# renjie-liang/HUAL

Measured on AMD Instinct MI355X. Metric: train clips/sec, higher is better.
Workload: dtype f32 (fp16x3 / bf16x3 split-operand MFMA, fp32 accumulate); 1 GPU; Charades-STA SeqPAN train step (fwd+bwd+clip+AdamWD, dropout 0.2), batch 64/GPU, T=128, vdim=1024, L=20, C=8, dim=128, 8 heads, 2 attention layers, random init; ONE batch resident in HBM, batch assembly (hual_assemble_batch) outside the timed region; global_batch=64, T=128, vdim=1024, L=20, parallelism=dp1, launch=hipGraph, video_dtype=f32

## Files before the change

hual_amd/csrc/heads.h:

```cpp
#pragma once
#include "common.h"
#include "rowops.h"

namespace hual {

enum { LA_MATCH_SUM = 0, LA_MASK_SUM = 1, LA_ORTHO = 2, LA_LOC = 3, LA_ALIGN = 4, LA_DENOM = 5 };

struct PoolArgs {
  const float* F2;
  const float* wp;
  const float* Wbot;
  float* alpha;
  float* pooled;
  float* PW;
};
struct AlignPool;
struct AlignPoolBwd;
int launch_pool_align_fwd(const PoolArgs& a, const AlignPool* ap, const RowSpace& rs, hipStream_t s);
struct PoolBwd {
  const float* dFuse;
  float* dPW;
  float* dF2;
  float* dwp;
};
int launch_pool_align_bwd(const PoolArgs& a, const PoolBwd& g, const AlignPool& ap, const AlignPoolBwd& ab, const RowSpace& rs, hipStream_t s);

struct MatchArgs {
  const float* fuse;
  const float* Wm;
  const float* bm;
  const float* E;
  const int32_t* labels;
  float* probs;
  float* probs2;
  float* outputs;
  float* loss_acc;
  float* part;
  const uint32_t* rng;
  float inv_tau;
};
int match_fwd_blocks(int Nv);
struct AlignSim;
int launch_match_fwd(const MatchArgs& a, const RowSpace& rs, const AlignSim* as, hipStream_t s);
struct LossTailArgs {
  float* loss_acc; const float* match_part; int match_nblk; const float* loc_part; int loc_nblk;
  float lambda, override_denom; const float* denom_dev; float* loss_out;
  const uint32_t* ovf; int novf;
  const float* align_rows; int nalign;
};
struct MatchBwd {
  const float* dOut;
  const float* dOut2;
  float* dFuse;
  float* dWm; float* dbm; float* dE;
  const float* dE_ortho;
  float* part;
  float lambda;
  int do_tail; LossTailArgs tail;
};
int match_bwd_blocks(int Nv);
int launch_match_bwd(const MatchArgs& a, const MatchBwd& g, const RowSpace& rs, hipStream_t s);
struct HeadsArgs {
  const float* h[2]; const float* w[2]; const float* b[2];
  float* logit[2];
  const float* vmask;
  const float* y1; const float* y2;
  int64_t* start_index; int64_t* end_index;
  float* ds; float* de;
  int grad_only;
  float* dZ[2];
  float* part[2];
  float* loc_part;
  float inv_batch;
  const uint32_t* ovf; int novf;
};
int launch_heads(const HeadsArgs& a, int B, int T, hipStream_t s);
int launch_loss_tail(const LossTailArgs& a, hipStream_t s);

struct AlignPool {
  const float* F2;
  const float* F1;
  const float* inner;
  float* tpre; float* vpre;
  float* that; float* vhat;
  int ld;
};
struct AlignSim {
  const float* that; const float* vhat; int Bg;
  float* dq; float* da;
  float* row_loss;
  float* dthat; float* dvhat;
  float* loss_acc;
  float scale;
  int ld;
  int row0, nrows;
};
int launch_align_sim(const AlignSim& a, hipStream_t s);
struct AlignPoolBwd {
  const float* dthat; const float* dvhat;
  float* dF2;
  float* dF1;
  const float* col_dq; const float* col_da; int col_Bg;
};

}
```

hual_amd/csrc/heads.hip:

```cpp
#include "heads.h"
#include "philox.h"
#include "prof.h"

using namespace hual;

#if defined(HUAL_STAMPS) && HUAL_STAMPS == 8
static __device__ unsigned long long g_heads_stamps[512 * 64];
extern "C" int hual_debug_stamps(unsigned long long* out, int n) {
  return (int)hipMemcpyFromSymbol(out, HIP_SYMBOL(g_heads_stamps), sizeof(unsigned long long) * (size_t)n);
}
#define HEADS_STAMP(i) do { if (threadIdx.x == 0 && blockIdx.x < 512) g_heads_stamps[blockIdx.x * 64 + (i)] = __builtin_readcyclecounter(); } while (0)
#else
#define HEADS_STAMP(i) do { } while (0)
#endif

__device__ __forceinline__ void pool_fwd_body(const PoolArgs& a, const RowSpace& rs, int b) {
  __shared__ float al[256];
  __shared__ float pooled[HUAL_D];
  __shared__ float part[HUAL_D];
  const int tid = threadIdx.x;
  const bool on = tid < 256;
  const int l32 = tid & 31, grp = tid >> 5;
  const int L = rs.L;
  const float* F = a.F2 + (size_t)(rs.Nv + b * L) * HUAL_D;
  const float* m = rs.rowmask + rs.Nv + b * L;
  if (on) {
    const float4 w4 = ld4(a.wp + 4 * l32);
    for (int l = grp; l < L; l += 8) {
      const float4 f = ld4(F + (size_t)l * HUAL_D + 4 * l32);
      const float d = fast_sum32(f.x * w4.x + f.y * w4.y + f.z * w4.z + f.w * w4.w);
      if (l32 == 0) al[l] = d * m[l] + HUAL_MASK_VALUE * (1.0f - m[l]);
    }
  }
  __syncthreads();
  float mx = -INFINITY;
  for (int l = 0; l < L; ++l) mx = fmaxf(mx, al[l]);
  float sum = 0.f;
  for (int l = 0; l < L; ++l) sum += __expf(al[l] - mx);
  const float inv = 1.0f / sum;
  const int c = tid & 127, half = (tid >> 7) & 1;
  if (on && half == 0) {
    float p = 0.f;
    for (int l = 0; l < L; ++l) {
      const float alpha = __expf(al[l] - mx) * inv;
      if (c == 0) a.alpha[b * L + l] = alpha;
      p = fmaf(alpha, F[(size_t)l * HUAL_D + c], p);
    }
    pooled[c] = p;
    a.pooled[b * HUAL_D + c] = p;
  }
  __syncthreads();
  float o = 0.f;
  if (on) {
#pragma unroll 8
// ... 15 lines not shown
  float ce_sum = 0.f, m_sum = 0.f;
  float4 w0 = ld4(a.Wm + (col + 0) * 4), w1 = ld4(a.Wm + (col + 1) * 4), w2 = ld4(a.Wm + (col + 2) * 4), w3 = ld4(a.Wm + (col + 3) * 4);
  const float4 bm = ld4(a.bm);
  float4 e0 = ld4(a.E + col), e1 = ld4(a.E + HUAL_D + col), e2 = ld4(a.E + 2 * HUAL_D + col), e3 = ld4(a.E + 3 * HUAL_D + col);
  uint3 gk = make_uint3(0u, 0u, 0u);
  if (a.rng) gk = make_uint3(a.rng[0], a.rng[1], a.rng[2]);
  for (int row = bid * 8 + grp; row < rs.Nv; row += nblk * 8) {
    const size_t off = (size_t)row * HUAL_D + col;
    const float4 f = ld4(a.fuse + off);
    float l0 = f.x * w0.x + f.y * w1.x + f.z * w2.x + f.w * w3.x;
    float l1 = f.x * w0.y + f.y * w1.y + f.z * w2.y + f.w * w3.y;
    float l2 = f.x * w0.z + f.y * w1.z + f.z * w2.z + f.w * w3.z;
    float l3 = f.x * w0.w + f.y * w1.w + f.z * w2.w + f.w * w3.w;
    l0 = fast_sum32(l0) + bm.x; l1 = fast_sum32(l1) + bm.y; l2 = fast_sum32(l2) + bm.z; l3 = fast_sum32(l3) + bm.w;
    if (a.rng) {
      const uint4_ r = philox4x32(0u, (uint32_t)row, (uint32_t)HUAL_SITE_GUMBEL, gk.z, gk.x, gk.y);
      l0 = (l0 + gumbel_noise(r.x)) * a.inv_tau; l1 = (l1 + gumbel_noise(r.y)) * a.inv_tau;
      l2 = (l2 + gumbel_noise(r.z)) * a.inv_tau; l3 = (l3 + gumbel_noise(r.w)) * a.inv_tau;
    }
    const float mx = fmaxf(fmaxf(l0, l1), fmaxf(l2, l3));
    const float x0 = expf(l0 - mx), x1 = expf(l1 - mx), x2 = expf(l2 - mx), x3 = expf(l3 - mx);
    const float sum = x0 + x1 + x2 + x3;
    const float inv = 1.0f / sum;
    const float p0 = x0 * inv, p1 = x1 * inv, p2 = x2 * inv, p3 = x3 * inv;
    const float mk = rs.rowmask[row];
    if (l32 == 0) {
      *reinterpret_cast<float4*>(a.probs + (size_t)row * 4) = make_float4(p0, p1, p2, p3);
      if (a.probs2) *reinterpret_cast<float4*>(a.probs2 + (size_t)row * 4) = make_float4(p0, p1, p2, p3);
      if (a.labels) {
        const int lab = a.labels[row];
        const float ll = lab == 0 ? l0 : (lab == 1 ? l1 : (lab == 2 ? l2 : l3));
        ce_sum += (mx + logf(sum) - ll) * mk;
        m_sum += mk;
      }
    }
    float4 o = make_float4((f.x + p0 * e0.x + p1 * e1.x + p2 * e2.x + p3 * e3.x) * mk,
                           (f.y + p0 * e0.y + p1 * e1.y + p2 * e2.y + p3 * e3.y) * mk,
                           (f.z + p0 * e0.z + p1 * e1.z + p2 * e2.z + p3 * e3.z) * mk,
                           (f.w + p0 * e0.w + p1 * e1.w + p2 * e2.w + p3 * e3.w) * mk);
    st4(a.outputs + off, o);
  }
  if (a.labels && a.loss_acc) {
    if (l32 == 0) { red[0][grp] = ce_sum; red[1][grp] = m_sum; }
    __syncthreads();
    if (threadIdx.x == 0) {
      float c = 0.f, m = 0.f;
      for (int i = 0; i < 8; ++i) { c += red[0][i]; m += red[1][i]; }
      if (a.part) { a.part[2 * bid] = c; a.part[2 * bid + 1] = m; }
      else { atomicAdd(a.loss_acc + LA_MATCH_SUM, c); atomicAdd(a.loss_acc + LA_MASK_SUM, m); }
    }
  }
}

__device__ __forceinline__ float loss_tail_body(const LossTailArgs& a, float* sm, bool write);
__global__ __launch_bounds__(256) void match_bwd_kernel(MatchArgs a, MatchBwd g, RowSpace rs) {
  __shared__ float4 red[8][8][32];
  __shared__ float redb[8][4];
  const int l32 = threadIdx.x & 31, grp = threadIdx.x >> 5;
  const int col = 4 * l32;
  float4 w0 = ld4(a.Wm + (col + 0) * 4), w1 = ld4(a.Wm + (col + 1) * 4), w2 = ld4(a.Wm + (col + 2) * 4), w3 = ld4(a.Wm + (col + 3) * 4);
  float4 e0 = ld4(a.E + col), e1 = ld4(a.E + HUAL_D + col), e2 = ld4(a.E + 2 * HUAL_D + col), e3 = ld4(a.E + 3 * HUAL_D + col);
  const int row0 = min((int)blockIdx.x * 8 + grp, rs.Nv - 1);
  const size_t off0 = (size_t)row0 * HUAL_D + col;
  float pmk = rs.rowmask[row0];
  float4 pd = ld4(g.dOut + off0), pd2 = g.dOut2 ? ld4(g.dOut2 + off0) : f4zero();
  float4 pf = ld4(a.fuse + off0), pp = *reinterpret_cast<const float4*>(a.probs + (size_t)row0 * 4);
  float denom = 1.0f;
  if (g.do_tail) {
    __shared__ float smt[12];
    denom = loss_tail_body(g.tail, smt, blockIdx.x == 0);
  } else if (a.labels) {
    denom = a.loss_acc[LA_DENOM];
  }
  const float ce_scale = a.labels ? g.lambda / denom : 0.f;
  float4 dE0 = f4zero(), dE1 = f4zero(), dE2 = f4zero(), dE3 = f4zero();
  float4 dW0 = f4zero(), dW1 = f4zero(), dW2 = f4zero(), dW3 = f4zero();
  float db0 = 0.f, db1 = 0.f, db2 = 0.f, db3 = 0.f;
  for (int row = blockIdx.x * 8 + grp; row < rs.Nv; row += gridDim.x * 8) {
    const size_t off = (size_t)row * HUAL_D + col;
    const float mk = pmk;
    float4 d = pd;
    if (g.dOut2) d = make_float4(d.x + pd2.x, d.y + pd2.y, d.z + pd2.z, d.w + pd2.w);
    const float4 f = pf, p = pp;
    {
      const int rn = min(row + (int)gridDim.x * 8, rs.Nv - 1);
      const size_t offn = (size_t)rn * HUAL_D + col;
      pmk = rs.rowmask[rn];
      pd = ld4(g.dOut + offn);
      if (g.dOut2) pd2 = ld4(g.dOut2 + offn);
      pf = ld4(a.fuse + offn);
      pp = *reinterpret_cast<const float4*>(a.probs + (size_t)rn * 4);
    }
    d = make_float4(d.x * mk, d.y * mk, d.z * mk, d.w * mk);
    float q0 = fast_sum32(d.x * e0.x + d.y * e0.y + d.z * e0.z + d.w * e0.w);
    float q1 = fast_sum32(d.x * e1.x + d.y * e1.y + d.z * e1.z + d.w * e1.w);
    float q2 = fast_sum32(d.x * e2.x + d.y * e2.y + d.z * e2.z + d.w * e2.w);
    float q3 = fast_sum32(d.x * e3.x + d.y * e3.y + d.z * e3.z + d.w * e3.w);
    const float dot = p.x * q0 + p.y * q1 + p.z * q2 + p.w * q3;
    float dl0 = p.x * (q0 - dot), dl1 = p.y * (q1 - dot), dl2 = p.z * (q2 - dot), dl3 = p.w * (q3 - dot);
    if (a.labels) {
      const int lab = a.labels[row];
      const float cs = ce_scale * mk;
      dl0 += cs * (p.x - (lab == 0 ? 1.f : 0.f));
      dl1 += cs * (p.y - (lab == 1 ? 1.f : 0.f));
      dl2 += cs * (p.z - (lab == 2 ? 1.f : 0.f));
      dl3 += cs * (p.w - (lab == 3 ? 1.f : 0.f));
    }
    if (a.rng) { dl0 *= a.inv_tau; dl1 *= a.inv_tau; dl2 *= a.inv_tau; dl3 *= a.inv_tau; }
    st4(g.dFuse + off, make_float4(d.x + dl0 * w0.x + dl1 * w0.y + dl2 * w0.z + dl3 * w0.w,
                                   d.y + dl0 * w1.x + dl1 * w1.y + dl2 * w1.z + dl3 * w1.w,
                                   d.z + dl0 * w2.x + dl1 * w2.y + dl2 * w2.z + dl3 * w2.w,
                                   d.w + dl0 * w3.x + dl1 * w3.y + dl2 * w3.z + dl3 * w3.w));
    dE0 = make_float4(dE0.x + p.x * d.x, dE0.y + p.x * d.y, dE0.z + p.x * d.z, dE0.w + p.x * d.w);
    dE1 = make_float4(dE1.x + p.y * d.x, dE1.y + p.y * d.y, dE1.z + p.y * d.z, dE1.w + p.y * d.w);
    dE2 = make_float4(dE2.x + p.z * d.x, dE2.y + p.z * d.y, dE2.z + p.z * d.z, dE2.w + p.z * d.w);
    dE3 = make_float4(dE3.x + p.w * d.x, dE3.y + p.w * d.y, dE3.z + p.w * d.z, dE3.w + p.w * d.w);
    dW0 = make_float4(dW0.x + f.x * dl0, dW0.y + f.y * dl0, dW0.z + f.z * dl0, dW0.w + f.w * dl0);
    dW1 = make_float4(dW1.x + f.x * dl1, dW1.y + f.y * dl1, dW1.z + f.z * dl1, dW1.w + f.w * dl1);
    dW2 = make_float4(dW2.x + f.x * dl2, dW2.y + f.y * dl2, dW2.z + f.z * dl2, dW2.w + f.w * dl2);
    dW3 = make_float4(dW3.x + f.x * dl3, dW3.y + f.y * dl3, dW3.z + f.z * dl3, dW3.w + f.w * dl3);
    if (l32 == 0) { db0 += dl0; db1 += dl1; db2 += dl2; db3 += dl3; }
  }
  red[0][grp][l32] = dE0; red[1][grp][l32] = dE1; red[2][grp][l32] = dE2; red[3][grp][l32] = dE3;
  red[4][grp][l32] = dW0; red[5][grp][l32] = dW1; red[6][grp][l32] = dW2; red[7][grp][l32] = dW3;
  if (l32 == 0) { redb[grp][0] = db0; redb[grp][1] = db1; redb[grp][2] = db2; redb[grp][3] = db3; }
  __syncthreads();
  float* part = g.part + (size_t)blockIdx.x * 9 * HUAL_D;
  for (int idx = threadIdx.x; idx < 8 * 128; idx += 256) {
    const int vec = idx >> 7, c = idx & 127;
    float s = 0.f;
#pragma unroll
    for (int k = 0; k < 8; ++k) s += reinterpret_cast<const float*>(&red[vec][k][c >> 2])[c & 3];
    if (vec < 4) {
      if (g.dE_ortho && blockIdx.x == 0) s += g.dE_ortho[vec * HUAL_D + c];
      part[vec * HUAL_D + c] = s;
    } else {
      part[4 * HUAL_D + c * 4 + (vec - 4)] = s;
    }
  }
  if (threadIdx.x < HUAL_D) {
    float s = 0.f;
    if (threadIdx.x < 4)
      for (int k = 0; k < 8; ++k) s += redb[k][threadIdx.x];
    part[8 * HUAL_D + threadIdx.x] = s;
  }
}

template <int NR>
__global__ __launch_bounds__(512) void heads_kernel(HeadsArgs a, int T, int B) {
  __shared__ float zs_[256], ze_[256], ps[256], pe[256], dls[256], dle[256];
  __shared__ float sm[24];
  __shared__ double smd[16];
  __shared__ float wtot[2][4];
  __shared__ float bestv[2][4];
  __shared__ int besti[2][4];
  __shared__ float4 red[2][16][32];
  __shared__ float redb[2][16];
  const int b = xcd_tile(blockIdx.x, gridDim.x), tid = threadIdx.x;
  if (b >= B) return;
  const int l32 = tid & 31, grp = tid >> 5;
  const int col = 4 * l32;
  HEADS_STAMP(0);
  float4 hs[NR], he[NR];
  float4 ws = f4zero(), we = f4zero();
  float poison = 0.f;
  if (a.ovf) {
    bool bad = false;
    for (int i = tid & 63; i < a.novf; i += 64) bad |= a.ovf[i] != 0u;
    if (__any(bad)) poison = __builtin_nanf("");
  }
  if (a.h[0]) {
    ws = ld4(a.w[0] + col); we = ld4(a.w[1] + col);
#pragma unroll
    for (int u = 0; u < NR; ++u) {
      const int t = min(grp + 16 * u, T - 1);
      hs[u] = ld4(a.h[0] + (size_t)(b * T + t) * HUAL_D + col);
      he[u] = ld4(a.h[1] + (size_t)(b * T + t) * HUAL_D + col);
    }
  }
  if (a.grad_only) {
    if (tid < T) { dls[tid] = a.ds[b * T + tid]; dle[tid] = a.de[b * T + tid]; }
  } else if (a.h[0]) {
    const float bs = a.b[0][0] + poison, be = a.b[1][0] + poison;
#pragma unroll
    for (int u = 0; u < NR; ++u) {
      const int t = grp + 16 * u;
      const float ds = fast_sum32(hs[u].x * ws.x + hs[u].y * ws.y + hs[u].z * ws.z + hs[u].w * ws.w) + bs;
// ... 66 lines not shown
      wave_best(ve, ie);
      if ((t & 63) == 0) { bestv[0][t >> 6] = vs; besti[0][t >> 6] = is; bestv[1][t >> 6] = ve; besti[1][t >> 6] = ie; }
    }
    __syncthreads();
    if (t == 0) {
      float v; int i;
      best_of_waves(bestv[0], besti[0], 4, v, i);
      a.start_index[b] = i;
      best_of_waves(bestv[1], besti[1], 4, v, i);
      a.end_index[b] = i;
      if (poison != poison || nanlogit) { a.start_index[b] = -1; a.end_index[b] = -1; }
    }
  } else {
    __syncthreads();
  }
  HEADS_STAMP(4);
  HEADS_STAMP(5);
  if (a.dZ[0] && (a.y1 || a.grad_only)) {
    float4 dws = f4zero(), dwe = f4zero();
    float dbs = 0.f, dbe = 0.f;
#pragma unroll
    for (int u = 0; u < NR; ++u) {
      const int tt = grp + 16 * u;
      if (tt >= T) continue;
      const size_t off = (size_t)(b * T + tt) * HUAL_D + col;
      const float dl0 = dls[tt], dl1 = dle[tt];
      st4(a.dZ[0] + off, make_float4(hs[u].x > 0.f ? dl0 * ws.x : 0.f, hs[u].y > 0.f ? dl0 * ws.y : 0.f, hs[u].z > 0.f ? dl0 * ws.z : 0.f,
                                     hs[u].w > 0.f ? dl0 * ws.w : 0.f));
      st4(a.dZ[1] + off, make_float4(he[u].x > 0.f ? dl1 * we.x : 0.f, he[u].y > 0.f ? dl1 * we.y : 0.f, he[u].z > 0.f ? dl1 * we.z : 0.f,
                                     he[u].w > 0.f ? dl1 * we.w : 0.f));
      dws = make_float4(dws.x + dl0 * hs[u].x, dws.y + dl0 * hs[u].y, dws.z + dl0 * hs[u].z, dws.w + dl0 * hs[u].w);
      dwe = make_float4(dwe.x + dl1 * he[u].x, dwe.y + dl1 * he[u].y, dwe.z + dl1 * he[u].z, dwe.w + dl1 * he[u].w);
      if (l32 == 0) { dbs += dl0; dbe += dl1; }
    }
    red[0][grp][l32] = dws; red[1][grp][l32] = dwe;
    if (l32 == 0) { redb[0][grp] = dbs; redb[1][grp] = dbe; }
    __syncthreads();
    if (tid < 256) {
      const int hd = tid >> 7, c = tid & 127;
      float sw = 0.f;
#pragma unroll
      for (int k = 0; k < 16; ++k) sw += reinterpret_cast<const float*>(&red[hd][k][c >> 2])[c & 3];
      float sb = 0.f;
      if (c == 0)
        for (int k = 0; k < 16; ++k) sb += redb[hd][k];
      float* part = a.part[hd] + (size_t)b * 2 * HUAL_D;
      part[c] = sw;
      part[HUAL_D + c] = sb;
    }
  }
  HEADS_STAMP(6);
}

__device__ __forceinline__ float loss_tail_body(const LossTailArgs& a, float* sm, bool write) {
  const int tid = threadIdx.x;
  float cs = 0.f, ms = 0.f, ls = 0.f;
  for (int i = tid; i < a.match_nblk; i += 256) { cs += a.match_part[2 * i]; ms += a.match_part[2 * i + 1]; }
  if (write)
    for (int i = tid; i < a.loc_nblk; i += 256) ls += a.loc_part[i];
  int bad = 0;
  if (write) {
    for (int i = tid; i < a.novf; i += 256) bad |= a.ovf[i] != 0u;
    bad = __syncthreads_or(bad);
  }
  block_reduce<BlockSumF>(cs, ms, ls, sm);
  const float denom = a.denom_dev ? *a.denom_dev : (a.override_denom > 0.f ? a.override_denom : ms + 1e-12f);
  if (write && tid == 0) {
    float* la = a.loss_acc;
    la[LA_MATCH_SUM] = cs; la[LA_MASK_SUM] = ms; la[LA_LOC] = ls;
    la[LA_DENOM] = denom;
    if (a.align_rows) {
      float l = 0.f;
      for (int i = 0; i < a.nalign; ++i) l += a.align_rows[i];
      la[LA_ALIGN] = l;
    }
    if (a.loss_out) {
      const float match = cs / denom + la[LA_ORTHO];
      const float align = la[LA_ALIGN];
      const float poison = bad ? __builtin_nanf("") : 0.f;
      a.loss_out[0] = ls + a.lambda * match + align + poison;
      a.loss_out[1] = ls + poison;
      a.loss_out[2] = match + poison;
      a.loss_out[3] = align + poison;
    }
  }
  return denom;
}
__global__ __launch_bounds__(256) void loss_tail_kernel(LossTailArgs a) {
  __shared__ float sm[12];
  loss_tail_body(a, sm, true);
}

#define L2_EPS 1e-12f
__device__ __forceinline__ void align_pool_body(const AlignPool& a, const RowSpace& rs, int b) {
  __shared__ float sm[8];
  __shared__ float part[2][4][HUAL_D];
  const int c = threadIdx.x & 127, grp = threadIdx.x >> 7;
  const int L = rs.L, T = rs.T;
  float tc = 0.f, vc = 0.f;
  for (int l = threadIdx.x; l < L; l += 512) tc += rs.rowmask[rs.Nv + b * L + l];
  for (int t = threadIdx.x; t < T; t += 512) vc += rs.rowmask[b * T + t];
  tc = block_reduce<BlockSumF>(tc, sm);
  vc = block_reduce<BlockSumF>(vc, sm);
  float ts = 0.f, vs = 0.f;
#pragma unroll 8
  for (int l = grp; l < L; l += 4) ts += a.F2[(size_t)(rs.Nv + b * L + l) * HUAL_D + c];
#pragma unroll 8
  for (int t = grp; t < T; t += 4) vs += a.F1[(size_t)(b * T + t) * HUAL_D + c] * (a.inner[b * T + t] / vc);
  part[0][grp][c] = ts;
  part[1][grp][c] = vs;
  __syncthreads();
  ts = part[0][0][c] + part[0][1][c] + part[0][2][c] + part[0][3][c];
  vs = part[1][0][c] + part[1][1][c] + part[1][2][c] + part[1][3][c];
  const float tp = ts / tc;
  const float tn = block_reduce<BlockSumF>(grp == 0 ? tp * tp : 0.f, sm);
// ... 221 lines not shown
  }
  part[grp][c] = dw;
  __syncthreads();
  if (grp == 0) atomicAdd(pb.dwp + c, (part[0][c] + part[1][c]) + (part[2][c] + part[3][c]));
}

namespace hual {

int launch_pool_align_fwd(const PoolArgs& a, const AlignPool* ap, const RowSpace& rs, hipStream_t s) {
  HUAL_REQUIRE(rs.L <= 256, "pool: L <= 256");
  AlignPool z{};
  HUAL_LAUNCH(0.0, 512.0 * (rs.Nq + (ap ? rs.R : 0) + 4.0 * rs.B), pool_align_fwd_kernel, dim3(xcd_round8(rs.B), ap ? 2 : 1), dim3(512), 0, s, a, ap ? *ap : z, rs);
  HUAL_CHECK_HIP(hipGetLastError());
  return 0;
}
int launch_pool_align_bwd(const PoolArgs& a, const PoolBwd& g, const AlignPool& ap, const AlignPoolBwd& ab, const RowSpace& rs, hipStream_t s) {
  HUAL_REQUIRE(rs.T <= 256 && rs.L <= 256, "pool_align_bwd: T, L <= 256");
  HUAL_REQUIRE(ab.dF2 == g.dF2, "pool_align_bwd: the two parts write the same query rows");
  const double pab = 512.0 * (3.0 * rs.Nv + 2.0 * rs.Nq);
#define PAB(KT, KL) HUAL_LAUNCH(0.0, pab, (pool_align_bwd_kernel<KT, KL>), dim3(xcd_round8(rs.B)), dim3(512), 0, s, a, g, ap, ab, rs)
  if (rs.T <= 128) {
    if (rs.L <= 32) PAB(32, 8); else if (rs.L <= 64) PAB(32, 16); else if (rs.L <= 128) PAB(32, 32); else PAB(64, 64);
  } else {
    if (rs.L <= 32) PAB(64, 8); else if (rs.L <= 64) PAB(64, 16); else if (rs.L <= 128) PAB(64, 32); else PAB(64, 64);
  }
#undef PAB
  HUAL_CHECK_HIP(hipGetLastError());
  return 0;
}
static int rowgrid(int R, int cap) {
  int g = cdiv(R, 8);
  return g < cap ? (g > 0 ? g : 1) : cap;
}
int match_fwd_blocks(int Nv) { return rowgrid(Nv, 512); }
int match_bwd_blocks(int Nv) { return rowgrid(Nv, 256); }
int launch_match_fwd(const MatchArgs& a, const RowSpace& rs, const AlignSim* as, hipStream_t s) {
  HUAL_REQUIRE(a.part != nullptr, "match_fwd: partial-sum scratch");
  const int nm = match_fwd_blocks(rs.Nv);
  AlignSim z{};
  if (as) {
    HUAL_REQUIRE(as->Bg >= 1 && as->Bg <= 1024 && as->ld >= HUAL_D && as->row0 == 0 && as->nrows == as->Bg, "align: global batch <= 1024");
    z = *as;
  }
  HUAL_LAUNCH(0.0, (1024.0 + 32.0) * rs.Nv, match_align_fwd_kernel, dim3(nm + (as ? as->Bg : 0)), dim3(256), 0, s, a, rs, z, nm);
  HUAL_CHECK_HIP(hipGetLastError());
  return 0;
}
int launch_match_bwd(const MatchArgs& a, const MatchBwd& g, const RowSpace& rs, hipStream_t s) {
  HUAL_REQUIRE(g.part != nullptr, "match_bwd: partial-sum scratch");
  HUAL_LAUNCH(0.0, 4.0 * 512.0 * rs.Nv, match_bwd_kernel, dim3(match_bwd_blocks(rs.Nv)), dim3(256), 0, s, a, g, rs);
  HUAL_CHECK_HIP(hipGetLastError());
  return 0;
}
int launch_heads(const HeadsArgs& a, int B, int T, hipStream_t s) {
  HUAL_REQUIRE(T >= 1 && T <= 256 && B >= 1, "heads: T <= 256");
  HUAL_REQUIRE(a.grad_only ? (a.ds && a.de && a.dZ[0]) : (a.logit[0] && a.logit[1] && a.vmask && a.start_index && a.end_index), "heads: null tensor");
  HUAL_REQUIRE(!a.h[0] || (a.h[1] && a.w[0] && a.w[1] && a.b[0] && a.b[1]), "heads: hidden layers incomplete");
  HUAL_REQUIRE(!a.dZ[0] || (a.dZ[1] && a.part[0] && a.part[1] && a.h[0]), "heads: gradient outputs incomplete");
  const double hb = (a.dZ[0] ? 4.0 : 2.0) * 512.0 * B * T + 16.0 * B * T;
  if (T <= 128) HUAL_LAUNCH(0.0, hb, heads_kernel<8>, dim3(xcd_round8(B)), dim3(512), 0, s, a, T, B);
  else HUAL_LAUNCH(0.0, hb, heads_kernel<16>, dim3(xcd_round8(B)), dim3(512), 0, s, a, T, B);
  HUAL_CHECK_HIP(hipGetLastError());
  return 0;
}
int launch_loss_tail(const LossTailArgs& a, hipStream_t s) {
  HUAL_REQUIRE(a.loss_acc && a.match_part && a.loc_part, "loss_tail: null");
  HUAL_LAUNCH(0.0, 0.0, loss_tail_kernel, dim3(1), dim3(256), 0, s, a);
  HUAL_CHECK_HIP(hipGetLastError());
  return 0;
}
int launch_align_sim(const AlignSim& a, hipStream_t s) {
  HUAL_REQUIRE(a.Bg >= 1 && a.Bg <= 1024, "align: global batch <= 1024");
  HUAL_REQUIRE(a.ld >= HUAL_D && a.row0 >= 0 && a.nrows >= 1 && a.row0 + a.nrows <= a.Bg, "align: row window / leading dimension");
  HUAL_LAUNCH(0.0, 0.0, align_sim_rows_kernel, dim3(a.Bg), dim3(256), 0, s, a);
  HUAL_LAUNCH(0.0, 0.0, align_sim_cols_kernel, dim3(a.nrows), dim3(256), 0, s, a);
  HUAL_CHECK_HIP(hipGetLastError());
  return 0;
}

}
```

hual_amd/csrc/prof.cpp:

```cpp
#include <stdlib.h>
#include "prof.h"
#include <map>
#include <string>
#include <vector>
#include <string.h>
#include "../../include/hual_seqpan.h"

namespace hual {

namespace {
struct Rec { std::string name; hipEvent_t a, b; double flops, bytes; };
struct Agg { std::string name; int64_t launches = 0; double usec = 0.0, flops = 0.0, bytes = 0.0; };
struct State {
  bool on = false;
  std::vector<Rec> recs;
  std::vector<Agg> aggs;
};
thread_local State g_prof;

std::string clean(const char* s) {
  std::string n(s);
  while (!n.empty() && (n.front() == '(' || n.front() == ' ')) n.erase(n.begin());
  while (!n.empty() && (n.back() == ')' || n.back() == ' ')) n.pop_back();
  return n;
// ... 19 lines not shown
}

extern "C" {

int hual_prof_begin(void) {
  hual::g_prof.on = true;
  hual::g_prof.recs.clear();
  hual::g_prof.aggs.clear();
  return 0;
}

int hual_prof_end(void) {
  using namespace hual;
  g_prof.on = false;
  std::map<std::string, size_t> idx;
  g_prof.aggs.clear();
  for (auto& r : g_prof.recs) {
    hipEventSynchronize(r.b);
    float ms = 0.f;
    const bool ok = hipEventElapsedTime(&ms, r.a, r.b) == hipSuccess;
    auto it = idx.find(r.name);
    if (it == idx.end()) {
      it = idx.emplace(r.name, g_prof.aggs.size()).first;
      g_prof.aggs.push_back(Agg{r.name});
    }
    Agg& a = g_prof.aggs[it->second];
    if (ok) { a.launches += 1; a.usec += (double)ms * 1e3; a.flops += r.flops; a.bytes += r.bytes; }
    hipEventDestroy(r.a);
    hipEventDestroy(r.b);
  }
  g_prof.recs.clear();
  return (int)g_prof.aggs.size();
}

int hual_prof_get(int i, char* name, int name_cap, int64_t* launches, double* usec, double* flops, double* bytes) {
  using namespace hual;
  if (i < 0 || i >= (int)g_prof.aggs.size() || !name || name_cap < 1) return HUAL_ERR_INVALID;
  const Agg& a = g_prof.aggs[i];
  strncpy(name, a.name.c_str(), (size_t)name_cap - 1);
  name[name_cap - 1] = 0;
  if (launches) *launches = a.launches;
  if (usec) *usec = a.usec;
  if (flops) *flops = a.flops;
  if (bytes) *bytes = a.bytes;
  return 0;
}

int hual_prof_kernel_pipe(const char* kernel, int* pipe, int* passes) {
  if (!kernel || !pipe || !passes) return HUAL_ERR_INVALID;
  struct Row { const char* prefix; int pipe, passes; };
  static const Row rows[] = {
      {"conv_block_", HUAL_PIPE_MATRIX16, 3}, {"ln_proj", HUAL_PIPE_MATRIX16, 3}, {"da_post", HUAL_PIPE_MATRIX16, 3},
      {"da_mid_bwd", HUAL_PIPE_MATRIX16, 3},  {"ln2_mid_bwd", HUAL_PIPE_MATRIX16, 3}, {"mproj_", HUAL_PIPE_MATRIX16, 3},
      {"feature_", HUAL_PIPE_MATRIX16, 3},    {"dw_f16_", HUAL_PIPE_MATRIX16, 3},
      {"attn_", HUAL_PIPE_MATRIX16, 3},      {"cq_fwd_staged", HUAL_PIPE_MATRIX16, 3}, {"cq_bwd_staged", HUAL_PIPE_MATRIX16, 3},
      {"cq_fwd_wide", HUAL_PIPE_MATRIX16, 3}, {"cq_bwd_wide", HUAL_PIPE_MATRIX16, 3},
      {"cq_", HUAL_PIPE_MATRIX32, 1},
  };
  for (const Row& r : rows)
    if (strncmp(kernel, r.prefix, strlen(r.prefix)) == 0) { *pipe = r.pipe; *passes = r.passes; return 0; }
  *pipe = HUAL_PIPE_NONE; *passes = 0;
  return 0;
}

}
```

hual_amd/csrc/seqpan.hip:

```cpp
#include "attn.h"
#include "prof.h"
#include "cq.h"
#include "convblock.h"
#include "dablock.h"
#include "embed.h"
#include "gemm.h"
#include "heads.h"
#include "mproj.h"
#include "optim.h"
#include "params.h"
#include "rowops.h"
#include <stdlib.h>
#include <string.h>
#include <algorithm>
#include <unordered_map>
#include <vector>

namespace hual {
const char* last_error_cstr();
}
using namespace hual;

namespace {

// ... 787 lines not shown
    pr.s[1] = mstep_reuse(c.nimg(pm.shid.k, 1), D, true, false);
    pr.s[2] = mstep(b.dz[1], D, D, c.nimg(pm.ehid.k, 1), D, false, true);    mstep_out(pr.s[2], g.d_out, D);
    pr.s[3] = mstep_reuse(c.nimg(pm.ehid.k, 0), D, true, true);             mstep_out(pr.s[3], g.d_fn[1], D);
    c.chk(launch_mproj(&pr, 1, c.drop, c.stream));
  }
  return g;
}

float* bwd_fe(Ctx& c, int ps, const HeadBufs& hd, float* d_fn, float* d_in) {
  const ParamMap& pm = c.pm;
  const int D = HUAL_D, Nv = c.rs.Nv;
  const std::string dt = "d.fe" + std::to_string(ps);
  const FeBufs b = fe_bufs(Res{c, false}, ps);
  float* f = b.cb.x[4];
  float* dzd = c.actv(dt + ".zd");
  c.push_dw(mkdw(b.l2, D, D, dzd, D, Nv, c.g(pm.fe_dense.k), c.g(pm.fe_dense.b)));
  float* d_res = c.actv(dt + ".res");
  float* d_att = c.actv(dt + ".att");
  {
    LnProjBwdArgs lb{};
    const LnP& hl = ps == 1 ? pm.eln : pm.sln;
    lb.pre_x = b.out; lb.pre_mean = hd.mean + (ps == 1 ? Nv : 0); lb.pre_rstd = hd.rstd + (ps == 1 ? Nv : 0);
    lb.pre_g = c.p(hl.g); lb.pre_dy = d_fn; lb.pre_add = ps == 1 ? nullptr : d_in;
    lb.a_bits[0] = b.kb8; lb.a_save[0] = dzd;
    lb.nsteps = 1; lb.A[0] = nullptr; lb.lda[0] = D; lb.wimg_t[0] = c.nimg(pm.fe_dense.k); lb.dst[0] = 0;
    lb.dy1_bits = b.kb7; lb.x = b.res; lb.mean = b.mean2; lb.rstd = b.rstd2; lb.g1 = c.p(pm.fe_ln2.g);
    lb.dx = d_res; lb.dz = d_att; lb.dz_bits = b.kb6; lb.R = Nv; lb.drop_row0 = 0;
    c.ln_proj_bwd(lb, c.g(pm.fe_ln2.g), c.g(pm.fe_ln2.b), c.g(hl.g), c.g(hl.b));
  }
  float* d_qkv = c.buf(dt + ".qkv", Nv, 3 * D);
  AttnJob a = b.job;
  a.dO = d_att; a.lddo = D; a.dQ = d_qkv; a.lddq = 3 * D; a.dK = d_qkv + D; a.dV = d_qkv + 2 * D; a.lddkv = 3 * D;
  c.attn_bwd(&a, 1);
  const DenseP* pr[3] = {&pm.fe_q, &pm.fe_k, &pm.fe_v};
  for (int k = 0; k < 3; ++k) c.push_dw(mkdw(b.a, D, D, d_qkv + k * D, 3 * D, Nv, c.g(pr[k]->k), c.g(pr[k]->b)));
  float* d_f = c.actv(dt + ".x4");
  {
    LnProjBwdArgs lb{};
    lb.nsteps = 3;
    for (int k = 0; k < 3; ++k) { lb.A[k] = d_qkv + k * D; lb.lda[k] = 3 * D; lb.wimg_t[k] = c.nimg(pr[k]->k); lb.dst[k] = 0; }
    lb.dy1_bits = b.kb4; lb.x = f; lb.mean = b.mean; lb.rstd = b.rstd; lb.g1 = c.p(pm.fe_ln1.g); lb.add1 = d_res;
    lb.dx = d_f; lb.R = Nv; lb.drop_row0 = 0;
    c.ln_proj_bwd(lb, c.g(pm.fe_ln1.g), c.g(pm.fe_ln1.b), nullptr, nullptr);
  }
  return conv_block_bwd(c, b.cb, d_f, pm.fe_cb, c.rsv);
}

float* bwd_fuse(Ctx& c, const CoreBufs& k, const FuseBufs& f, const HeadBufs& hd, float* cqf, float* d_in, float* d_out_heads,
                const hual_labels* lab, const hual_run_opts* opt) {
  const ParamMap& pm = c.pm;
  const int D = HUAL_D, Nv = c.rs.Nv, B = c.B;
  c.stage(ST_FUSE);
  float* d_fuse = c.actv("d.fuse");
  float* match_part_b = c.buf("part." + std::to_string(c.part_seq++), (size_t)match_bwd_blocks(Nv) * 9, D);
  ColsumJob cj{};
  cj.src = match_part_b; cj.nblk = match_bwd_blocks(Nv); cj.nvec = 9; cj.last_ncols = 4;
  for (int i = 0; i < 4; ++i) { cj.dst[i] = c.g(pm.label_emb) + i * D; cj.dst[4 + i] = c.g(pm.match.k) + i * D; }
  cj.dst[8] = c.g(pm.match.b);
  if (c.active) c.colsum.push_back(cj);
  if (c.live()) {
    MatchArgs ma = match_args(c, k, f, lab, opt);
    ma.probs = f.probs;
    MatchBwd mb{};
    mb.dOut = d_in; mb.dOut2 = d_out_heads; mb.dFuse = d_fuse; mb.dWm = c.g(pm.match.k); mb.dbm = c.g(pm.match.b); mb.dE = c.g(pm.label_emb);
    mb.lambda = c.cfg->match_lambda;
    mb.dE_ortho = k.ortho_dE;
    mb.part = match_part_b;
    if (opt->deferred_loss_terms && c.sel_stage < 0) {
      mb.do_tail = 1;
      mb.tail = LossTailArgs{k.loss_acc, f.match_part, match_fwd_blocks(Nv), hd.loc_part, B, c.cfg->match_lambda,
                             opt->match_denom_override, opt->match_denom_dev, opt->deferred_loss_terms, k.ovf, c.novf,
                             opt->align_external ? nullptr : f.align_rows, B};
    }
    c.chk(launch_match_bwd(ma, mb, c.rs, c.stream));
  }
  float* d_cqf = c.act("d.cq.feats");
  c.push_dw(mkdw(cqf, D, D, d_fuse, D, Nv, c.g(pm.cqcat.k), c.g(pm.cqcat.b)));
  if (c.live()) {
    MProjArgs pr = margs(Nv); pr.nsteps = 1;
    pr.s[0] = mstep(d_fuse, D, D, c.nimg(pm.cqcat.k), D, true, true);
    mstep_out(pr.s[0], d_cqf, D);
    c.chk(launch_mproj(&pr, 1, c.drop, c.stream));
  }
  float* d_pw = c.buf("d.pool.pw", B, D);
  if (c.live()) {
    AlignPoolBwd ab{f.d_that, f.d_vhat, d_cqf, d_cqf, nullptr, nullptr, 0};
    if (!opt->align_external && c.sel_stage < 0) {
      ab.col_dq = f.align_scratch; ab.col_da = f.align_scratch + (size_t)B * B; ab.col_Bg = B;
    }
    PoolBwd pb{d_fuse, d_pw, d_cqf, c.g(pm.pool_w)};
    c.chk(launch_pool_align_bwd(f.pool, pb, f.align, ab, c.rs, c.stream));
  }
  c.push_dw(mkdw(f.pool.pooled, D, D, d_pw, D, B, c.g(pm.cqcat.k) + (size_t)D * D, nullptr));
  return d_cqf;
}

float* bwd_cq(Ctx& c, const CqStage& q, float* d_cqf) {
  const ParamMap& pm = c.pm;
  const int D = HUAL_D, Nv = c.rs.Nv, Nq = c.rs.Nq, B = c.B, T = c.T, L = c.L;
  const CqBufs& cq = q.b;
  const float* xf = cq.X;
  c.stage(ST_CQ);
  for (int s = 0; s < 2; ++s) {
    const size_t ro = s == 0 ? 0 : (size_t)Nv * D;
    DwJob j = mkdw(xf + ro, D, D, d_cqf + ro, D, s == 0 ? Nv : Nq, c.g(pm.cq[s].dense), nullptr);
    j.npieces = 4;
    const float* a1[4] = {xf + ro, cq.C2Q + ro, xf + ro, xf + ro};
    const float* a2[4] = {nullptr, nullptr, cq.C2Q + ro, cq.Q2C + ro};
    for (int p = 0; p < 4; ++p) {
      j.A[p] = a1[p]; j.A2[p] = a2[p]; j.lda[p] = D; j.lda2[p] = D; j.kw[p] = D;
      j.dW[p] = c.g(pm.cq[s].dense) + (size_t)p * D * D;
    }
    c.push_dw(j);
  }
  CqBwdBufs cg{};
  cg.dCat = nullptr; cg.ldcat = 4 * D; cg.dC2Q = c.act("d.cq.c2q"); cg.dQ2C = c.act("d.cq.q2c"); cg.dX = c.act("d.cq.x");
  if (c.live()) {
    MProjArgs pr[2];
    for (int sd = 0; sd < 2; ++sd) {
      const size_t ro = sd == 0 ? 0 : (size_t)Nv;
      pr[sd] = margs(sd == 0 ? Nv : Nq, sd == 0 ? Nq : Nv);
      pr[sd].nsteps = 4;
      for (int p = 0; p < 4; ++p) {
        const float* img = c.nimg(pm.cq[sd].dense, p);
        pr[sd].s[p] = p == 0 ? mstep(d_cqf + ro * D, D, D, img, D, true, true) : mstep_reuse(img, D, true, true);
      }
      pr[sd].quad_x = xf + ro * D; pr[sd].quad_c2q = cq.C2Q + ro * D; pr[sd].quad_q2c = cq.Q2C + ro * D;
      pr[sd].quad_dc2q = cg.dC2Q + ro * D; pr[sd].quad_dq2c = cg.dQ2C + ro * D; pr[sd].quad_dx = cg.dX + ro * D;
    }
    c.chk(launch_mproj(pr, 2, c.drop, c.stream));
  }
  cg.dD1W = c.act("d.cq.d1w"); cg.dD2 = c.act("d.cq.d2"); cg.dS0 = c.vec("d.cq.s0"); cg.dS1 = c.vec("d.cq.s1");
  cg.dM2 = c.buf("d.cq.m2", (size_t)2 * B * cq_m2_rows_host(T, L), D);
  cg.GD = cq_bwd_global(B, T, L) ? c.buf("d.cq.gd", (size_t)4 * B, cq_mat_elems_host(T, L)) : nullptr;
  float *dXa = c.act("d.cq.xa"), *dXb = c.act("d.cq.xb");
// ... 487 lines not shown
```

Measured before the change: 53890 clips/s.

## Fuse match backward with cqcat input-gradient projection in one kernel

Adds a fuse_bwd kernel that computes the match-head backward (dFuse, dE/dW/db partials) and then immediately multiplies the freshly computed dFuse tile by the cqcat weight via MFMA from LDS to produce d_cqf. This replaces the separate match_bwd and mproj launches when the tile count allows. It aims to save one launch and one round-trip of dFuse through HBM. The loss-tail reduction moves into dedicated head blocks. The cost is higher register and LDS use per block and a different partial-sum block count.

```diff
diff --git a/hual_amd/csrc/heads.h b/hual_amd/csrc/heads.h
--- a/hual_amd/csrc/heads.h
+++ b/hual_amd/csrc/heads.h
@@ -60,6 +60,13 @@
 };
 int match_bwd_blocks(int Nv);
 int launch_match_bwd(const MatchArgs& a, const MatchBwd& g, const RowSpace& rs, hipStream_t s);
+struct FuseBwdProd {
+  const float* wimg;
+  float* dX;
+  int MT;
+};
+int fuse_bwd_blocks(int Nv, int MT);
+int launch_fuse_bwd(const MatchArgs& a, const MatchBwd& g, const FuseBwdProd& x, const RowSpace& rs, hipStream_t s);
 struct HeadsArgs {
   const float* h[2]; const float* w[2]; const float* b[2];
   float* logit[2];
diff --git a/hual_amd/csrc/heads.hip b/hual_amd/csrc/heads.hip
--- a/hual_amd/csrc/heads.hip
+++ b/hual_amd/csrc/heads.hip
@@ -1,5 +1,6 @@
 #include "heads.h"
 #include "philox.h"
+#include "tilecore.h"
 #include "prof.h"
 
 using namespace hual;
@@ -121,6 +122,7 @@
   }
 }
 
+template <int NTH = 256>
 __device__ __forceinline__ float loss_tail_body(const LossTailArgs& a, float* sm, bool write);
 __global__ __launch_bounds__(256) void match_bwd_kernel(MatchArgs a, MatchBwd g, RowSpace rs) {
   __shared__ float4 red[8][8][32];
@@ -202,6 +204,150 @@
     for (int k = 0; k < 8; ++k) s += reinterpret_cast<const float*>(&red[vec][k][c >> 2])[c & 3];
     if (vec < 4) {
       if (g.dE_ortho && blockIdx.x == 0) s += g.dE_ortho[vec * HUAL_D + c];
+      part[vec * HUAL_D + c] = s;
+    } else {
+      part[4 * HUAL_D + c * 4 + (vec - 4)] = s;
+    }
+  }
+  if (threadIdx.x < HUAL_D) {
+    float s = 0.f;
+    if (threadIdx.x < 4)
+      for (int k = 0; k < 8; ++k) s += redb[k][threadIdx.x];
+    part[8 * HUAL_D + threadIdx.x] = s;
+  }
+}
+
+#define FB_ROWS 64
+#define FB_HEAD 8
+#define FB_LDS (2 * FB_ROWS * 256 + 8 * 8 * 32 * 16)
+template <int NT>
+__global__ __launch_bounds__(CB_THREADS) void fuse_bwd_kernel(MatchArgs a, MatchBwd g, FuseBwdProd x, RowSpace rs) {
+  extern __shared__ __attribute__((aligned(16))) char fb_lds[];
+  char* S = fb_lds;
+  float4* red = reinterpret_cast<float4*>(fb_lds + 2 * FB_ROWS * 256);
+  __shared__ float redb[8][4];
+  __shared__ float ainv[FB_ROWS];
+  const int lane = threadIdx.x & 63, wave = threadIdx.x >> 6;
+  const int l32 = threadIdx.x & 31, grp = threadIdx.x >> 5;
+  const int col = 4 * l32;
+  const int MT = x.MT, Nv = rs.Nv;
+  const int head = g.do_tail ? FB_HEAD : 0;
+  if ((int)blockIdx.x < head) {
+    if (blockIdx.x == 0) {
+      __shared__ float smh[24];
+      loss_tail_body<CB_THREADS>(g.tail, smh, true);
+    }
+    return;
+  }
+  const int tile = xcd_tile(blockIdx.x - head, gridDim.x - head);
+  const int r0 = tile * MT;
+  if (r0 >= Nv) return;
+  const int RE = min(Nv, r0 + MT);
+  TfW wc;
+  tf_load_w(wc, x.wimg, wave, lane);
+  const float* d2p = g.dOut2 ? g.dOut2 : g.dOut;
+  const int32_t* labp = a.labels ? a.labels : reinterpret_cast<const int32_t*>(rs.rowmask);
+  float rmk[NT];
+  float4 rd[NT], rd2[NT], rf[NT], rp[NT];
+  int rlab[NT];
+#pragma unroll
+  for (int u = 0; u < NT; ++u) {
+    const int row = min(r0 + grp + 16 * u, RE - 1);
+    const size_t off = (size_t)row * HUAL_D + col;
+    rmk[u] = rs.rowmask[row];
+    rd[u] = ld4(g.dOut + off);
+    rd2[u] = ld4(d2p + off);
+    rf[u] = ld4(a.fuse + off);
+    rp[u] = *reinterpret_cast<const float4*>(a.probs + (size_t)row * 4);
+    rlab[u] = labp[row];
+  }
+  float4 w0 = ld4(a.Wm + (col + 0) * 4), w1 = ld4(a.Wm + (col + 1) * 4), w2 = ld4(a.Wm + (col + 2) * 4), w3 = ld4(a.Wm + (col + 3) * 4);
+  float4 e0 = ld4(a.E + col), e1 = ld4(a.E + HUAL_D + col), e2 = ld4(a.E + 2 * HUAL_D + col), e3 = ld4(a.E + 3 * HUAL_D + col);
+  float denom = 1.0f;
+  if (g.do_tail) {
+    __shared__ float smt[24];
+    denom = loss_tail_body<CB_THREADS>(g.tail, smt, false);
+  } else if (a.labels) {
+    denom = a.loss_acc[LA_DENOM];
+  }
+  const float ce_scale = a.labels ? g.lambda / denom : 0.f;
+  float4 dE0 = f4zero(), dE1 = f4zero(), dE2 = f4zero(), dE3 = f4zero();
+  float4 dW0 = f4zero(), dW1 = f4zero(), dW2 = f4zero(), dW3 = f4zero();
+  float db0 = 0.f, db1 = 0.f, db2 = 0.f, db3 = 0.f;
+#pragma unroll
+  for (int u = 0; u < NT; ++u) {
+    const int lr = grp + 16 * u, row = r0 + lr;
+    const bool ok = lr < MT && row < RE;
+    const float mk = rmk[u];
+    float4 d = rd[u];
+    if (g.dOut2) d = make_float4(d.x + rd2[u].x, d.y + rd2[u].y, d.z + rd2[u].z, d.w + rd2[u].w);
+    const float4 f = rf[u], p = rp[u];
+    d = make_float4(d.x * mk, d.y * mk, d.z * mk, d.w * mk);
+    float q0 = fast_sum32(d.x * e0.x + d.y * e0.y + d.z * e0.z + d.w * e0.w);
+    float q1 = fast_sum32(d.x * e1.x + d.y * e1.y + d.z * e1.z + d.w * e1.w);
+    float q2 = fast_sum32(d.x * e2.x + d.y * e2.y + d.z * e2.z + d.w * e2.w);
+    float q3 = fast_sum32(d.x * e3.x + d.y * e3.y + d.z * e3.z + d.w * e3.w);
+    const float dot = p.x * q0 + p.y * q1 + p.z * q2 + p.w * q3;
+    float dl0 = p.x * (q0 - dot), dl1 = p.y * (q1 - dot), dl2 = p.z * (q2 - dot), dl3 = p.w * (q3 - dot);
+    if (a.labels) {
+      const int lab = rlab[u];
+      const float cs = ce_scale * mk;
+      dl0 += cs * (p.x - (lab == 0 ? 1.f : 0.f));
+      dl1 += cs * (p.y - (lab == 1 ? 1.f : 0.f));
+      dl2 += cs * (p.z - (lab == 2 ? 1.f : 0.f));
+      dl3 += cs * (p.w - (lab == 3 ? 1.f : 0.f));
+    }
+    if (a.rng) { dl0 *= a.inv_tau; dl1 *= a.inv_tau; dl2 *= a.inv_tau; dl3 *= a.inv_tau; }
+    const float4 df = make_float4(d.x + dl0 * w0.x + dl1 * w0.y + dl2 * w0.z + dl3 * w0.w,
+                                  d.y + dl0 * w1.x + dl1 * w1.y + dl2 * w1.z + dl3 * w1.w,
+                                  d.z + dl0 * w2.x + dl1 * w2.y + dl2 * w2.z + dl3 * w2.w,
+                                  d.w + dl0 * w3.x + dl1 * w3.y + dl2 * w3.z + dl3 * w3.w);
+    if (ok) {
+      st4(g.dFuse + (size_t)row * HUAL_D + col, df);
+      dE0 = make_float4(dE0.x + p.x * d.x, dE0.y + p.x * d.y, dE0.z + p.x * d.z, dE0.w + p.x * d.w);
+      dE1 = make_float4(dE1.x + p.y * d.x, dE1.y + p.y * d.y, dE1.z + p.y * d.z, dE1.w + p.y * d.w);
+      dE2 = make_float4(dE2.x + p.z * d.x, dE2.y + p.z * d.y, dE2.z + p.z * d.z, dE2.w + p.z * d.w);
+      dE3 = make_float4(dE3.x + p.w * d.x, dE3.y + p.w * d.y, dE3.z + p.w * d.z, dE3.w + p.w * d.w);
+      dW0 = make_float4(dW0.x + f.x * dl0, dW0.y + f.y * dl0, dW0.z + f.z * dl0, dW0.w + f.w * dl0);
+      dW1 = make_float4(dW1.x + f.x * dl1, dW1.y + f.y * dl1, dW1.z + f.z * dl1, dW1.w + f.w * dl1);
+      dW2 = make_float4(dW2.x + f.x * dl2, dW2.y + f.y * dl2, dW2.z + f.z * dl2, dW2.w + f.w * dl2);
+      dW3 = make_float4(dW3.x + f.x * dl3, dW3.y + f.y * dl3, dW3.z + f.z * dl3, dW3.w + f.w * dl3);
+      if (l32 == 0) { db0 += dl0; db1 += dl1; db2 += dl2; db3 += dl3; }
+    }
+    const float inv = cb_store_operand(S, S + FB_ROWS * 256, lr, l32, f4_pick(ok, df, f4zero()));
+    if (l32 == 0) ainv[lr] = row < RE ? inv : 0.f;
+  }
+  {
+    auto fold = [&](int v, const float4& t) {
+      const float4 o = make_float4(t.x + lane_xor32(t.x, lane), t.y + lane_xor32(t.y, lane), t.z + lane_xor32(t.z, lane), t.w + lane_xor32(t.w, lane));
+      if (lane < 32) red[(v * 8 + wave) * 32 + l32] = o;
+    };
+    fold(0, dE0); fold(1, dE1); fold(2, dE2); fold(3, dE3);
+    fold(4, dW0); fold(5, dW1); fold(6, dW2); fold(7, dW3);
+    db0 += lane_xor32(db0, lane); db1 += lane_xor32(db1, lane); db2 += lane_xor32(db2, lane); db3 += lane_xor32(db3, lane);
+    if (lane == 0) { redb[wave][0] = db0; redb[wave][1] = db1; redb[wave][2] = db2; redb[wave][3] = db3; }
+  }
+  lds_barrier();
+  {
+    const int j = lane & 15, gq = lane >> 4, ecol = 16 * wave + 4 * gq;
+    f32x4 accp[NT];
+    tf_mma<NT, FB_ROWS * 256>(S, wc, lane, accp);
+#pragma unroll
+    for (int rt = 0; rt < NT; ++rt) {
+      const int row = r0 + 16 * rt + j;
+      const float ir = ainv[16 * rt + j];
+      const float4 v = make_float4(fmaf(accp[rt][0], ir, 0.f), fmaf(accp[rt][1], ir, 0.f), fmaf(accp[rt][2], ir, 0.f), fmaf(accp[rt][3], ir, 0.f));
+      if (16 * rt + j < MT && row < RE) st4(x.dX + (size_t)row * HUAL_D + ecol, v);
+    }
+  }
+  float* part = g.part + (size_t)tile * 9 * HUAL_D;
+  for (int idx = threadIdx.x; idx < 8 * 128; idx += CB_THREADS) {
+    const int vec = idx >> 7, c = idx & 127;
+    float s = 0.f;
+#pragma unroll
+    for (int k = 0; k < 8; ++k) s += reinterpret_cast<const float*>(&red[(vec * 8 + k) * 32 + (c >> 2)])[c & 3];
+    if (vec < 4) {
+      if (g.dE_ortho && tile == 0) s += g.dE_ortho[vec * HUAL_D + c];
       part[vec * HUAL_D + c] = s;
     } else {
       part[4 * HUAL_D + c * 4 + (vec - 4)] = s;
@@ -374,15 +520,17 @@
   HEADS_STAMP(6);
 }
 
+template <int NTH>
 __device__ __forceinline__ float loss_tail_body(const LossTailArgs& a, float* sm, bool write) {
   const int tid = threadIdx.x;
+  const bool on = NTH <= 256 || tid < 256;
   float cs = 0.f, ms = 0.f, ls = 0.f;
-  for (int i = tid; i < a.match_nblk; i += 256) { cs += a.match_part[2 * i]; ms += a.match_part[2 * i + 1]; }
+  for (int i = tid; on && i < a.match_nblk; i += 256) { cs += a.match_part[2 * i]; ms += a.match_part[2 * i + 1]; }
   if (write)
-    for (int i = tid; i < a.loc_nblk; i += 256) ls += a.loc_part[i];
+    for (int i = tid; on && i < a.loc_nblk; i += 256) ls += a.loc_part[i];
   int bad = 0;
   if (write) {
-    for (int i = tid; i < a.novf; i += 256) bad |= a.ovf[i] != 0u;
+    for (int i = tid; on && i < a.novf; i += 256) bad |= a.ovf[i] != 0u;
     bad = __syncthreads_or(bad);
   }
   block_reduce<BlockSumF>(cs, ms, ls, sm);
@@ -710,6 +858,24 @@
   HUAL_CHECK_HIP(hipGetLastError());
   return 0;
 }
+int fuse_bwd_blocks(int Nv, int MT) { return cdiv(Nv, MT); }
+int launch_fuse_bwd(const MatchArgs& a, const MatchBwd& g, const FuseBwdProd& x, const RowSpace& rs, hipStream_t s) {
+  HUAL_REQUIRE(g.part != nullptr, "fuse_bwd: partial-sum scratch");
+  HUAL_REQUIRE(x.wimg && x.dX && x.MT >= 1 && x.MT <= FB_ROWS && rs.Nv >= 1, "fuse_bwd: product");
+  const int grid = xcd_round8(fuse_bwd_blocks(rs.Nv, x.MT)) + (g.do_tail ? FB_HEAD : 0);
+  const int nt = (x.MT + 15) / 16;
+  const double flops = 2.0 * rs.Nv * 128.0 * 128.0;
+  const double bytes = 512.0 * rs.Nv * (g.dOut2 ? 5.0 : 4.0) + 24.0 * rs.Nv + 65536.0;
+#define FUSE_BWD(NT)                                                                                          \
+  do {                                                                                                        \
+    HUAL_DYN_LDS((fuse_bwd_kernel<NT>), 96 * 1024);                                                           \
+    HUAL_LAUNCH(flops, bytes, (fuse_bwd_kernel<NT>), dim3(grid), dim3(CB_THREADS), FB_LDS, s, a, g, x, rs);  \
+  } while (0)
+  if (nt <= 1) FUSE_BWD(1); else if (nt == 2) FUSE_BWD(2); else if (nt == 3) FUSE_BWD(3); else FUSE_BWD(4);
+#undef FUSE_BWD
+  HUAL_CHECK_HIP(hipGetLastError());
+  return 0;
+}
 int launch_heads(const HeadsArgs& a, int B, int T, hipStream_t s) {
   HUAL_REQUIRE(T >= 1 && T <= 256 && B >= 1, "heads: T <= 256");
   HUAL_REQUIRE(a.grad_only ? (a.ds && a.de && a.dZ[0]) : (a.logit[0] && a.logit[1] && a.vmask && a.start_index && a.end_index), "heads: null tensor");
diff --git a/hual_amd/csrc/prof.cpp b/hual_amd/csrc/prof.cpp
--- a/hual_amd/csrc/prof.cpp
+++ b/hual_amd/csrc/prof.cpp
@@ -95,7 +95,7 @@
   static const Row rows[] = {
       {"conv_block_", HUAL_PIPE_MATRIX16, 3}, {"ln_proj", HUAL_PIPE_MATRIX16, 3}, {"da_post", HUAL_PIPE_MATRIX16, 3},
       {"da_mid_bwd", HUAL_PIPE_MATRIX16, 3},  {"ln2_mid_bwd", HUAL_PIPE_MATRIX16, 3}, {"mproj_", HUAL_PIPE_MATRIX16, 3},
-      {"feature_", HUAL_PIPE_MATRIX16, 3},    {"dw_f16_", HUAL_PIPE_MATRIX16, 3},
+      {"feature_", HUAL_PIPE_MATRIX16, 3},    {"dw_f16_", HUAL_PIPE_MATRIX16, 3},     {"fuse_bwd_", HUAL_PIPE_MATRIX16, 3},
       {"attn_", HUAL_PIPE_MATRIX16, 3},      {"cq_fwd_staged", HUAL_PIPE_MATRIX16, 3}, {"cq_bwd_staged", HUAL_PIPE_MATRIX16, 3},
       {"cq_fwd_wide", HUAL_PIPE_MATRIX16, 3}, {"cq_bwd_wide", HUAL_PIPE_MATRIX16, 3},
       {"cq_", HUAL_PIPE_MATRIX32, 1},
diff --git a/hual_amd/csrc/seqpan.hip b/hual_amd/csrc/seqpan.hip
--- a/hual_amd/csrc/seqpan.hip
+++ b/hual_amd/csrc/seqpan.hip
@@ -863,16 +863,23 @@
   const int D = HUAL_D, Nv = c.rs.Nv, B = c.B;
   c.stage(ST_FUSE);
   float* d_fuse = c.actv("d.fuse");
+  const int chain_mt = mproj_rows(Nv);
+  bool chain = c.sel_stage < 0 && !opt->align_external && fuse_bwd_blocks(Nv, chain_mt) <= match_bwd_blocks(Nv);
+#ifdef HUAL_NO_FUSE_BWD_CHAIN
+  chain = false;
+#endif
+  const int match_nblk = chain ? fuse_bwd_blocks(Nv, chain_mt) : match_bwd_blocks(Nv);
   float* match_part_b = c.buf("part." + std::to_string(c.part_seq++), (size_t)match_bwd_blocks(Nv) * 9, D);
   ColsumJob cj{};
-  cj.src = match_part_b; cj.nblk = match_bwd_blocks(Nv); cj.nvec = 9; cj.last_ncols = 4;
+  cj.src = match_part_b; cj.nblk = match_nblk; cj.nvec = 9; cj.last_ncols = 4;
   for (int i = 0; i < 4; ++i) { cj.dst[i] = c.g(pm.label_emb) + i * D; cj.dst[4 + i] = c.g(pm.match.k) + i * D; }
   cj.dst[8] = c.g(pm.match.b);
   if (c.active) c.colsum.push_back(cj);
+  MatchArgs ma{};
+  MatchBwd mb{};
   if (c.live()) {
-    MatchArgs ma = match_args(c, k, f, lab, opt);
+    ma = match_args(c, k, f, lab, opt);
     ma.probs = f.probs;
-    MatchBwd mb{};
     mb.dOut = d_in; mb.dOut2 = d_out_heads; mb.dFuse = d_fuse; mb.dWm = c.g(pm.match.k); mb.dbm = c.g(pm.match.b); mb.dE = c.g(pm.label_emb);
     mb.lambda = c.cfg->match_lambda;
     mb.dE_ortho = k.ortho_dE;
@@ -883,15 +890,20 @@
                              opt->match_denom_override, opt->match_denom_dev, opt->deferred_loss_terms, k.ovf, c.novf,
                              opt->align_external ? nullptr : f.align_rows, B};
     }
-    c.chk(launch_match_bwd(ma, mb, c.rs, c.stream));
+    if (!chain) c.chk(launch_match_bwd(ma, mb, c.rs, c.stream));
   }
   float* d_cqf = c.act("d.cq.feats");
   c.push_dw(mkdw(cqf, D, D, d_fuse, D, Nv, c.g(pm.cqcat.k), c.g(pm.cqcat.b)));
   if (c.live()) {
-    MProjArgs pr = margs(Nv); pr.nsteps = 1;
-    pr.s[0] = mstep(d_fuse, D, D, c.nimg(pm.cqcat.k), D, true, true);
-    mstep_out(pr.s[0], d_cqf, D);
-    c.chk(launch_mproj(&pr, 1, c.drop, c.stream));
+    if (chain) {
+      FuseBwdProd fp{c.nimg(pm.cqcat.k), d_cqf, chain_mt};
+      c.chk(launch_fuse_bwd(ma, mb, fp, c.rs, c.stream));
+    } else {
+      MProjArgs pr = margs(Nv); pr.nsteps = 1;
+      pr.s[0] = mstep(d_fuse, D, D, c.nimg(pm.cqcat.k), D, true, true);
+      mstep_out(pr.s[0], d_cqf, D);
+      c.chk(launch_mproj(&pr, 1, c.drop, c.stream));
+    }
   }
   float* d_pw = c.buf("d.pool.pw", B, D);
   if (c.live()) {
```

After: 54370 clips/s, median of 6. No clear change (+0.9%).
